# danielSanchezQ/dkg

Measured on AMD Instinct MI355X. Metric: verified shares/sec (whole node) at n=1024,t=511; full-ceremony wall time, higher is better.
Workload: dtype u32 (GF(2^255-19), Z_l); 1 GPU; one DKG ceremony n=1024, t=511 (share gen + round-2/4 checks + finalise); n=1024, t=511, parallelism=single GPU, verify_streams=2, rounds_2_4_fused=True, degree_split=4, recombination=short lattice multipliers, recombination_addends=affine Niels, stepping_additions=dedicated (complete redo where exceptional)

## Files before the change

### dkg_amd/csrc/ge25519.h

```cpp
#pragma once
#include "fe25519.h"

struct ge_p3 {
  fe X, Y, Z, T;
};
struct ge_cached {
  fe YpX, YmX, Z2, T2d;
};
struct ge_aff {
  fe ypx, ymx, xy2d;
};

namespace ge_const {
__device__ static const uint32_t D[10] = {0x35978a3u, 0xd37284u, 0x3156ebdu, 0x6a0a0eu, 0x1c029u,
                                          0x179e898u, 0x3a03cbbu, 0x1ce7198u, 0x2e2b6ffu, 0x1480db3u};
__device__ static const uint32_t D2[10] = {0x2b2f159u, 0x1a6e509u, 0x22add7au, 0xd4141du, 0x38052u,
                                           0xf3d130u, 0x3407977u, 0x19ce331u, 0x1c56dffu, 0x901b67u};
__device__ static const uint32_t D4[10] = {0x165e2b2u, 0x14dca13u, 0x55baf5u, 0x1a8283bu, 0x700a4u,
                                           0x1e7a260u, 0x280f2eeu, 0x139c663u, 0x38adbffu, 0x12036ceu};
__device__ static const uint32_t D16[10] = {0x1978aeeu, 0x137284du, 0x156ebd6u, 0xa0a0ecu, 0x1c0293u,
                                            0x19e8980u, 0x203cbbbu, 0xe7198eu, 0x22b6ffeu, 0x80db3bu};
__device__ static const uint32_t SQRT_M1[10] = {0x20ea0b0u, 0x186c9d2u, 0x8f189du, 0x35697fu,
                                                0xbd0c60u, 0x1fbd7a7u, 0x2804c9eu, 0x1e16569u,
                                                0x4fc1du, 0xae0c92u};
__device__ static const uint32_t SQRT_AD_MINUS_ONE[10] = {
    0x17b2e1bu, 0x1fda812u, 0x297afd2u, 0x60dbc2u, 0x2be7638u,
    0x1f5d1fdu, 0x27e6498u, 0x11581e7u, 0x3f2b834u, 0xdda4c6u};
__device__ static const uint32_t INVSQRT_A_MINUS_D[10] = {
    0x5d40eau, 0x3f6aa0u, 0x257d339u, 0xbad20bu, 0x274bc58u,
    0x1d840u, 0x13dc8ffu, 0x19442d8u, 0x5cfaffu, 0x1e1b224u};
__device__ static const uint32_t ONE_MINUS_D_SQ[10] = {
    0x5fc176u, 0x1027065u, 0x2a1fc4fu, 0x1c66af1u, 0xb20684u,
    0x70dfe4u, 0x255eedfu, 0x1af332u, 0x28b2b3eu, 0xa41cau};
__device__ static const uint32_t D_MINUS_ONE_SQ[10] = {
    0xed4d20u, 0x156aa91u, 0x3332635u, 0x16580f0u, 0x34a7928u,
    0x9b4eebu, 0x26997a9u, 0x48299bu, 0x3af66c2u, 0x165a2cdu};
}

DKG_DEV void fe_ld(fe& r, const uint32_t* c) {
#pragma unroll
  for (int i = 0; i < 10; i++) r.v[i] = c[i];
}

DKG_DEV void ge_identity(ge_p3& p) {
  fe_zero(p.X);
  fe_one(p.Y);
  fe_one(p.Z);
  fe_zero(p.T);
}

DKG_DEV void ge_to_cached(ge_cached& c, const ge_p3& p) {
  fe_add(c.YpX, p.Y, p.X);
  fe_sub(c.YmX, p.Y, p.X);
  fe_dbl(c.Z2, p.Z);
  fe d2;
  fe_ld(d2, ge_const::D2);
  fe_mul(c.T2d, p.T, d2);
}

DKG_DEV void ge_cached_neg(ge_cached& r, const ge_cached& c) {
  fe_copy(r.YpX, c.YmX);
  fe_copy(r.YmX, c.YpX);
  fe_copy(r.Z2, c.Z2);
  fe_neg(r.T2d, c.T2d);
  fe_carry(r.T2d, r.T2d);
}

template <bool IL = false>
DKG_DEV void ge_add(ge_p3& r, const ge_p3& p, const ge_cached& q) {
  if constexpr (IL && DKG_PW) {
    fe a, b, e, h, t, u;
    fe_sub(t, p.Y, p.X);
    fe_add(u, p.Y, p.X);
    fe_mul2(a, t, q.YmX, b, u, q.YpX);
    fe_sub(e, b, a);
    fe_add(h, b, a);
    fe_mul2(a, p.T, q.T2d, b, p.Z, q.Z2);
    fe_sub(t, b, a);
    fe_add(b, b, a);
    fe_mul2(r.X, e, t, r.Y, b, h);
    fe_mul2(r.Z, b, t, r.T, e, h);
    return;
  }
  fe a, b, e, h, t;
  fe_sub(t, p.Y, p.X);
  fe_mul(a, t, q.YmX);
  fe_add(t, p.Y, p.X);
  fe_mul(b, t, q.YpX);
  fe_sub(e, b, a);
  fe_add(h, b, a);
  fe_mul(a, p.T, q.T2d);
  fe_mul(b, p.Z, q.Z2);
  fe_sub(t, b, a);
  fe_add(b, b, a);
  fe_mul(r.X, e, t);
  fe_mul(r.Y, b, h);
  fe_mul(r.Z, b, t);
  fe_mul(r.T, e, h);
}

DKG_DEV void ge_sub(ge_p3& r, const ge_p3& p, const ge_cached& q) {
  fe a, b, e, h, t;
  fe_sub(t, p.Y, p.X);
  fe_mul(a, t, q.YpX);
// ... 144 lines not shown
    fe_add(h, a, b);
    fe_sub(g, a, b);
    fe_add(a, p.X, p.Y);
    fe_sq2(t, p.Z, a, a);
    fe_dbl(t, t);
    fe_add(t, t, g);
    fe_carry(t, t);
    fe_sub(b, h, a);
    fe_mul2(r.X, b, t, r.Y, g, h);
    if (with_t) fe_mul2(r.Z, g, t, r.T, b, h);
    else fe_mul(r.Z, g, t);
    return;
  }
  fe a, b, t, h, g;
  fe_sq(a, p.X);
  fe_sq(b, p.Y);
  fe_add(h, a, b);
  fe_sub(g, a, b);
  fe_sq(t, p.Z);
  fe_dbl(t, t);
  fe_add(t, t, g);
  fe_carry(t, t);
  fe_add(a, p.X, p.Y);
  fe_sq(a, a);
  fe_sub(b, h, a);
  fe_mul(r.X, b, t);
  fe_mul(r.Y, g, h);
  fe_mul(r.Z, g, t);
  if (with_t) fe_mul(r.T, b, h);
}

template <bool IL = false>
DKG_DEV void ge_add_signed(ge_p3& r, const ge_p3& p, const ge_cached& q, bool neg, bool with_t = true) {
  fe a, b, e, h, t, qa, qb;
#pragma unroll
  for (int i = 0; i < 10; i++) {
    qa.v[i] = neg ? q.YpX.v[i] : q.YmX.v[i];
    qb.v[i] = neg ? q.YmX.v[i] : q.YpX.v[i];
  }
  if constexpr (IL && DKG_PW) {
    fe u;
    fe_sub(t, p.Y, p.X);
    fe_add(u, p.Y, p.X);
    fe_mul2(a, t, qa, b, u, qb);
  } else {
    fe_sub(t, p.Y, p.X);
    fe_mul(a, t, qa);
    fe_add(t, p.Y, p.X);
    fe_mul(b, t, qb);
  }
  fe_sub(e, b, a);
  fe_add(h, b, a);
  if constexpr (IL && DKG_PW) {
    fe_mul2(a, p.T, q.T2d, b, p.Z, q.Z2);
  } else {
    fe_mul(a, p.T, q.T2d);
    fe_mul(b, p.Z, q.Z2);
  }
  fe na;
  fe_neg(na, a);
  fe_cmov(a, na, neg);
  fe_sub(t, b, a);
  fe_add(b, b, a);
  if constexpr (IL && DKG_PW) {
    fe_mul2(r.X, e, t, r.Y, b, h);
    if (with_t) fe_mul2(r.Z, b, t, r.T, e, h);
    else fe_mul(r.Z, b, t);
  } else {
    fe_mul(r.X, e, t);
    fe_mul(r.Y, b, h);
    fe_mul(r.Z, b, t);
    if (with_t) fe_mul(r.T, e, h);
  }
}

template <bool IL = false>
DKG_DEV void ge_madd_signed(ge_p3& r, const ge_p3& p, const ge_aff& q, bool neg, bool with_t = true) {
  fe a, b, e, h, t, qa, qb;
#pragma unroll
  for (int i = 0; i < 10; i++) {
    qa.v[i] = neg ? q.ypx.v[i] : q.ymx.v[i];
    qb.v[i] = neg ? q.ymx.v[i] : q.ypx.v[i];
  }
  if constexpr (IL && DKG_PW) {
    fe u;
    fe_sub(t, p.Y, p.X);
    fe_add(u, p.Y, p.X);
    fe_mul2(a, t, qa, b, u, qb);
  } else {
    fe_sub(t, p.Y, p.X);
    fe_mul(a, t, qa);
    fe_add(t, p.Y, p.X);
    fe_mul(b, t, qb);
  }
  fe_sub(e, b, a);
  fe_add(h, b, a);
  fe_mul(a, p.T, q.xy2d);
  fe na;
  fe_neg(na, a);
  fe_cmov(a, na, neg);
  fe_dbl(b, p.Z);
  fe_carry(b, b);
  fe_sub(t, b, a);
  fe_add(b, b, a);
  if constexpr (IL && DKG_PW) {
    fe_mul2(r.X, e, t, r.Y, b, h);
    if (with_t) fe_mul2(r.Z, b, t, r.T, e, h);
    else fe_mul(r.Z, b, t);
  } else {
    fe_mul(r.X, e, t);
    fe_mul(r.Y, b, h);
    fe_mul(r.Z, b, t);
    if (with_t) fe_mul(r.T, e, h);
  }
}

template <bool IL = false>
DKG_DEV void ge_madd_swapped(ge_p3& r, const ge_p3& p, const ge_aff& q, bool neg, bool with_t = true) {
  fe a, b, e, h, t;
  const fe& qa = q.ymx;
  const fe& qb = q.ypx;
  if constexpr (IL && DKG_PW) {
    fe u;
    fe_sub(t, p.Y, p.X);
    fe_add(u, p.Y, p.X);
    fe_mul2(a, t, qa, b, u, qb);
  } else {
    fe_sub(t, p.Y, p.X);
    fe_mul(a, t, qa);
    fe_add(t, p.Y, p.X);
    fe_mul(b, t, qb);
  }
  fe_sub(e, b, a);
  fe_add(h, b, a);
  fe_mul(a, p.T, q.xy2d);
  fe na;
  fe_neg(na, a);
  fe_cmov(a, na, neg);
  fe_dbl(b, p.Z);
  fe_carry(b, b);
  fe_sub(t, b, a);
  fe_add(b, b, a);
  if constexpr (IL && DKG_PW) {
    fe_mul2(r.X, e, t, r.Y, b, h);
    if (with_t) fe_mul2(r.Z, b, t, r.T, e, h);
    else fe_mul(r.Z, b, t);
  } else {
    fe_mul(r.X, e, t);
    fe_mul(r.Y, b, h);
    fe_mul(r.Z, b, t);
    if (with_t) fe_mul(r.T, e, h);
  }
}


DKG_DEV bool fe_sqrt_ratio_m1(fe& r, const fe& u, const fe& v) {
  fe v3, v7, t, chk, neg_u, neg_u_i, sqrtm1;
  fe_ld(sqrtm1, ge_const::SQRT_M1);
  fe_sq(v3, v);
  fe_mul(v3, v3, v);
  fe_sq(v7, v3);
  fe_mul(v7, v7, v);
  fe_mul(t, u, v7);
  fe_pow22523(t, t);
  fe_mul(t, t, v3);
  fe_mul(r, t, u);
  fe_sq(chk, r);
  fe_mul(chk, chk, v);
  fe_neg(neg_u, u);
  fe_carry(neg_u, neg_u);
  fe_mul(neg_u_i, neg_u, sqrtm1);
  fe d;
  fe_sub(d, chk, u);
  bool correct = fe_iszero(d);
  fe_sub(d, chk, neg_u);
  bool flipped = fe_iszero(d);
  fe_sub(d, chk, neg_u_i);
  bool flipped_i = fe_iszero(d);
  fe r_prime;
  fe_mul(r_prime, r, sqrtm1);
  fe_cmov(r, r_prime, flipped || flipped_i);
  fe_abs(r, r);
  return correct || flipped;
}

DKG_DEV void fe_sq_x2(fe (&r)[2], const fe (&a)[2]) { fe_sq2(r[0], a[0], r[1], a[1]); }
DKG_DEV void fe_mul_x2(fe (&r)[2], const fe (&a)[2], const fe (&b)[2]) {
  fe_mul2(r[0], a[0], b[0], r[1], a[1], b[1]);
}
DKG_DEV void fe_sqn_x2(fe (&r)[2], const fe (&a)[2], int n) {
  fe_sq_x2(r, a);
  for (int i = 1; i < n; i++) fe_sq_x2(r, r);
}
DKG_DEV void fe_pow22523_x2(fe (&out)[2], const fe (&z)[2]) {
  fe t0[2], t1[2], t2[2];
  fe_sq_x2(t0, z);
  fe_sqn_x2(t1, t0, 2);
  fe_mul_x2(t1, z, t1);
  fe_mul_x2(t0, t0, t1);
  fe_sq_x2(t0, t0);
  fe_mul_x2(t0, t1, t0);
  fe_sqn_x2(t1, t0, 5);
  fe_mul_x2(t0, t1, t0);
  fe_sqn_x2(t1, t0, 10);
// ... 201 lines not shown
```

### dkg_amd/csrc/kernels.hip

```cpp
#ifdef DKG_FE_ILP
#define dkgk dkgk_ilp
#endif
#include "kernels.h"
#include "split.h"

#include <algorithm>
#include <cmath>
#include <type_traits>
#include "points.h"

namespace dkgk {

constexpr int COMB_WORDS = AFF_WORDS * COMB_ENTRIES;

#ifndef DKG_DECODE_WAVES
#define DKG_DECODE_WAVES 2
#endif
__global__ __launch_bounds__(256, DKG_DECODE_WAVES) void k_decode(const uint32_t* __restrict__ comp, size_t count,
                                                uint32_t* __restrict__ ext, size_t stride,
                                                uint8_t* __restrict__ ok, size_t pm_N, size_t pm_npad,
                                                uint32_t nseg, uint32_t seg, size_t pm_L, size_t pm_pstride) {
  size_t e = (size_t)blockIdx.x * blockDim.x + threadIdx.x;
  if (e >= count) return;
  uint32_t w[8];
// ... 1712 lines not shown
  const uint32_t* dw = digits + j * 256;
  const uint32_t* dw1 = digits + (nrecv + j) * 256;
  const int tp = top[j];
  ge_p3 acc;
  ge_identity(acc);
#pragma unroll 1
  for (int b = tp; b >= 0; b--) {
    uint64_t w = (uint32_t)__builtin_amdgcn_readfirstlane(dw[b]);
    if constexpr (K > 4) w |= (uint64_t)(uint32_t)__builtin_amdgcn_readfirstlane(dw1[b]) << 32;
    if (b != tp) ge_dbl_lean<DKG_AFF_IL != 0>(acc, acc, w != 0 || b == 0);
    aff_position<0, K, KL>(acc, w, qs, qr, b == 0);
  }
  if (live) pt_store_aos<DKG_COMB_NT != 0>(R, c * nrecv + j, acc);
}

void combine_short_aff(size_t width, size_t pstride, size_t pieces, size_t nrecv, const uint32_t* digits,
                       const int16_t* top, const uint32_t* A, uint32_t* R, hipStream_t stream, size_t j0, size_t jn) {
  if (!jn) jn = nrecv - j0;
  if (!width || !jn || pieces < 2 || pieces > 5) return;
  const dim3 grid((unsigned)((width + 63) / 64), (unsigned)jn);
  if (pieces == 2)
    hipLaunchKernelGGL((k_combine_aff<2, 1>), grid, dim3(64), 0, stream, width, pstride, nrecv, digits, top, A, R, j0);
  else if (pieces == 3)
    hipLaunchKernelGGL((k_combine_aff<3, 2>), grid, dim3(64), 0, stream, width, pstride, nrecv, digits, top, A, R, j0);
  else if (pieces == 4)
    hipLaunchKernelGGL((k_combine_aff<4, 2>), grid, dim3(64), 0, stream, width, pstride, nrecv, digits, top, A, R, j0);
  else
    hipLaunchKernelGGL((k_combine_aff<5, 2>), grid, dim3(64), 0, stream, width, pstride, nrecv, digits, top, A, R, j0);
}

constexpr int AFFQ_RUN = 32;

DKG_DEV void ld_zt(fe& z, fe& t, const uint32_t* R, size_t e) {
  const uint4* p4 = reinterpret_cast<const uint4*>(R + e * PT_WORDS) + 5;
  const uint4 a = p4[0], b = p4[1], c = p4[2], d = p4[3], f = p4[4];
  z = fe{{a.x, a.y, a.z, a.w, b.x, b.y, b.z, b.w, c.x, c.y}};
  t = fe{{c.z, c.w, d.x, d.y, d.z, d.w, f.x, f.y, f.z, f.w}};
}
DKG_DEV void ld_xy(fe& x, fe& y, const uint32_t* R, size_t e) {
  const uint4* p4 = reinterpret_cast<const uint4*>(R + e * PT_WORDS);
  const uint4 a = p4[0], b = p4[1], c = p4[2], d = p4[3], f = p4[4];
  x = fe{{a.x, a.y, a.z, a.w, b.x, b.y, b.z, b.w, c.x, c.y}};
  y = fe{{c.z, c.w, d.x, d.y, d.z, d.w, f.x, f.y, f.z, f.w}};
}
template <bool SC>
DKG_DEV void pair_fg(fe& z01, fe& f, fe& g, const fe& z0, const fe& t0, const fe& z1, const fe& t1, const fe& dc) {
  fe c, d;
  fe_mul(z01, z0, z1);
  fe_mul(c, t0, t1);
  fe_mul(c, c, dc);
  if constexpr (SC) {
    fe_copy(d, z01);
  } else {
    fe_dbl(d, z01);
    fe_carry(d, d);
  }
  fe_sub(f, d, c);
  fe_add(g, d, c);
}
DKG_DEV void st_niels(uint32_t* slot, const fe& x, const fe& y, const fe& d2) {
  fe ypx, ymx, t;
  fe_mul(t, x, y);
  fe_mul(t, t, d2);
  fe_add(ypx, y, x);
  fe_sub(ymx, y, x);
  st_fe3(slot, ypx, ymx, t);
}

template <bool SC>
__global__ __launch_bounds__(256) __attribute__((amdgpu_waves_per_eu(2, 2))) void k_affine_pairs(size_t width, size_t pstride, size_t pieces, size_t nrecv,
                                                      const uint32_t* __restrict__ R, uint32_t* __restrict__ A,
                                                      size_t j0, size_t jn, unsigned ls, unsigned rl) {
  const size_t span = (size_t)ls * rl, runs = (jn + span - 1) / span;
  const size_t gid = (size_t)blockIdx.x * blockDim.x + threadIdx.x;
  const size_t item = gid / ls;
  if (item >= (pieces / 2) * width * runs) return;
  const size_t c = item % width, rest = item / width, run = rest % runs, p = rest / runs;
  const size_t plane = pstride * nrecv;
  const size_t e0 = (2 * p * pstride + c) * nrecv + j0;
  const size_t jb = run * span + (gid % ls);
  const int cnt = jb < jn ? (int)min((size_t)rl, (jn - jb + ls - 1) / ls) : 0;
  auto pt = [&](int i) { return e0 + jb + ls * (size_t)i; };
  fe d2, dc;
  fe_ld(d2, ge_const::D2);
  fe_ld(dc, SC ? ge_const::D16 : ge_const::D2);
  fe acc;
  fe_one(acc);
#pragma unroll 1
  for (int i = 0; i < cnt; i++) {
    uint4* a4 = reinterpret_cast<uint4*>(A + pt(i) * AFFP_WORDS);
    a4[0] = make_uint4(acc.v[0], acc.v[1], acc.v[2], acc.v[3]);
    a4[1] = make_uint4(acc.v[4], acc.v[5], acc.v[6], acc.v[7]);
    a4[2] = make_uint4(acc.v[8], acc.v[9], 0u, 0u);
    fe z0, t0, z1, t1, z01, f, g;
    ld_zt(z0, t0, R, pt(i));
    ld_zt(z1, t1, R, pt(i) + plane);
    pair_fg<SC>(z01, f, g, z0, t0, z1, t1, dc);
    fe_mul(acc, acc, z01);
    fe_mul(f, f, g);
    fe_mul(acc, acc, f);
  }
  fe inv;
  fe_invert(inv, acc);
  if constexpr (SC) {
    fe_dbl(inv, inv);
    fe_carry(inv, inv);
  }
#pragma unroll 1
  for (int i = cnt - 1; i >= 0; i--) {
    const size_t e = pt(i);
    uint32_t* slot = A + e * AFFP_WORDS;
    fe z0, t0, z1, t1, z01, f, g, zs, iz0, iz1;
    ld_zt(z0, t0, R, e);
    ld_zt(z1, t1, R, e + plane);
    pair_fg<SC>(z01, f, g, z0, t0, z1, t1, dc);
    fe_mul(zs, f, g);
    {
      const uint4* a4 = reinterpret_cast<const uint4*>(slot);
      const uint4 q0 = a4[0], q1 = a4[1], q2 = a4[2];
      const fe pre = {{q0.x, q0.y, q0.z, q0.w, q1.x, q1.y, q1.z, q1.w, q2.x, q2.y}};
      fe t, i01;
      fe_mul(t, inv, pre);
      fe_mul(inv, inv, z01);
      fe_mul(inv, inv, zs);
      fe_mul(i01, t, zs);
      fe_mul(zs, t, z01);
      fe_mul(iz0, i01, z1);
      fe_mul(iz1, i01, z0);
    }
    fe_mul(f, f, zs);
    fe_mul(g, g, zs);
    fe ym0, yp0, ym1, yp1;
    {
      fe X, Y, x, y;
      ld_xy(X, Y, R, e);
      fe_sub(ym0, Y, X);
      fe_add(yp0, Y, X);
      fe_mul(x, X, iz0);
      fe_mul(y, Y, iz0);
      st_niels(slot, x, y, d2);
      ld_xy(X, Y, R, e + plane);
      fe_sub(ym1, Y, X);
      fe_add(yp1, Y, X);
      fe_mul(x, X, iz1);
      fe_mul(y, Y, iz1);
      st_niels(slot + plane * AFFP_WORDS, x, y, d2);
    }
    fe a, b, eh, x, y;
    fe_mul(a, ym0, ym1);
    fe_mul(b, yp0, yp1);
    fe_sub(eh, b, a);
    fe_mul(x, eh, f);
    fe_add(eh, b, a);
    fe_mul(y, eh, g);
    st_niels(slot + pieces * plane * AFFP_WORDS, x, y, d2);
    fe_mul(a, ym0, yp1);
    fe_mul(b, yp0, ym1);
    fe_sub(eh, b, a);
    fe_mul(x, eh, g);
    fe_add(eh, b, a);
    fe_mul(y, eh, f);
    st_niels(slot + (pieces + 1) * plane * AFFP_WORDS, x, y, d2);
  }
}

void affine_pairs(size_t width, size_t pstride, size_t pieces, size_t nrecv, const uint32_t* R, uint32_t* A,
                  hipStream_t stream, size_t j0, size_t jn, bool scaled) {
  if (!jn) jn = nrecv - j0;
  if (!width || !jn || pieces < 2) return;
  unsigned rl = AFFQ_RUN;
  while (rl > 8 && (pieces / 2) * width * ((jn + rl - 1) / rl) < 65536) rl /= 2;
  unsigned ls = 32;
  while (ls > 1 && (size_t)(ls / 2) * rl >= jn) ls /= 2;
  const size_t runs = (jn + (size_t)ls * rl - 1) / ((size_t)ls * rl), lanes = (pieces / 2) * width * runs * ls;
  hipLaunchKernelGGL(scaled ? k_affine_pairs<true> : k_affine_pairs<false>, dim3((unsigned)((lanes + 255) / 256)),
                     dim3(256), 0, stream, width, pstride, pieces, nrecv, R, A, j0, jn, ls, rl);
}

DKG_DEV void jsf_fetch(ge_aff& q, const uint32_t* __restrict__ A0, uint32_t slot, size_t plane, uint32_t e) {
  if (e == JSF_EV_NONE) return;
  asm volatile("" : "+v"(slot));
  const uint32_t* a = A0 + (size_t)slot * AFFP_WORDS + (e & 3u) * plane;
  const uint2* f0 = reinterpret_cast<const uint2*>(a + ((e & 4u) ? 10 : 0));
  const uint2* f1 = reinterpret_cast<const uint2*>(a + ((e & 4u) ? 0 : 10));
  const uint2* f2 = reinterpret_cast<const uint2*>(a + 20);
#pragma unroll
  for (int i = 0; i < 5; i++) {
    const uint2 u = f0[i], v = f1[i], w = f2[i];
    q.ypx.v[2 * i] = u.x;
    q.ypx.v[2 * i + 1] = u.y;
    q.ymx.v[2 * i] = v.x;
    q.ymx.v[2 * i + 1] = v.y;
    q.xy2d.v[2 * i] = w.x;
    q.xy2d.v[2 * i + 1] = w.y;
  }
}

struct JsfStream {
  ge_aff q;
  const uint32_t* A0;
  uint32_t slot;
  size_t plane;
  const uint32_t* ev;
  uint32_t next;
  int k;
};

template <int P, int K, int KL>
DKG_DEV void jsf_position(ge_p3& acc, uint32_t w, const uint32_t* qs, const ge_aff* qr, JsfStream& s, bool last) {
  if constexpr (2 * P < K) {
    const int e0 = (int8_t)(w >> (16 * P)), e1 = (int8_t)(w >> (16 * P + 8));
    bool t = last;
    if constexpr (2 * P + 2 < K) t = t || (w >> (16 * P + 16)) != 0;
    if (e0 != 0 && e1 != 0) {
      ge_madd_swapped<DKG_AFF_IL != 0>(acc, acc, s.q, e0 < 0, t);
      const uint32_t e = s.next;
      s.next = (uint32_t)__builtin_amdgcn_readfirstlane(s.ev[s.k]);
      s.k++;
      jsf_fetch(s.q, s.A0, s.slot, s.plane, e);
    } else if (e0 != 0 || e1 != 0) {
      constexpr int U0 = 2 * P, U1 = 2 * P + 1;
      if constexpr (U1 < KL) {
        const int u = e0 != 0 ? U0 : U1;
        ge_madd_lds<DKG_AFF_IL != 0>(acc, acc, qs + u * AFF_WORDS * 64 + threadIdx.x, (e0 | e1) < 0, 64, t);
      } else if (e0 != 0) {
        if constexpr (U0 < KL) ge_madd_lds<DKG_AFF_IL != 0>(acc, acc, qs + U0 * AFF_WORDS * 64 + threadIdx.x, e0 < 0, 64, t);
        else ge_madd_signed<DKG_AFF_IL != 0>(acc, acc, qr[U0 - KL], e0 < 0, t);
      } else {
        ge_madd_signed<DKG_AFF_IL != 0>(acc, acc, qr[U1 - KL], e1 < 0, t);
      }
    }
    jsf_position<P + 1, K, KL>(acc, w, qs, qr, s, last);
  }
}

template <int K, int KL>
__global__ __launch_bounds__(64, 2) void k_combine_jsf(size_t width, size_t pstride, size_t nrecv,
                                                       const uint32_t* __restrict__ digits,
                                                       const int16_t* __restrict__ top,
                                                       const uint32_t* __restrict__ ev,
                                                       const uint32_t* __restrict__ A, uint32_t* __restrict__ R,
                                                       size_t j0) {
  static_assert(K % 2 == 0 && K <= 4, "whole pairs in one digit word");
  __shared__ uint32_t qs[KL * AFF_WORDS * 64];
  const size_t c = (size_t)blockIdx.x * 64 + threadIdx.x;
  const size_t j = j0 + blockIdx.y;
  const bool live = c < width;
  const size_t cc = live ? c : 0;
  ge_aff qr[K - KL > 0 ? K - KL : 1];
  aff_addends<0, K, KL>(qs, qr, A, pstride, cc, nrecv, j);
  const uint32_t* dw = digits + j * 256;
  const int tp = top[j];
  JsfStream s;
  s.A0 = A + ((size_t)K * pstride * nrecv + j) * AFFP_WORDS;
  s.slot = (uint32_t)(cc * nrecv);
  s.plane = pstride * nrecv * AFFP_WORDS;
  s.ev = ev + j * JSF_EV_WORDS;
  s.next = (uint32_t)__builtin_amdgcn_readfirstlane(s.ev[1]);
  s.k = 2;
#pragma unroll
  for (int u = 0; u < K - KL; u++) {
#pragma unroll
    for (int i = 0; i < 10; i++)
      asm volatile("" : "+v"(qr[u].ypx.v[i]), "+v"(qr[u].ymx.v[i]), "+v"(qr[u].xy2d.v[i]));
  }
  fe_zero(s.q.ypx);
  fe_zero(s.q.ymx);
  fe_zero(s.q.xy2d);
  jsf_fetch(s.q, s.A0, s.slot, s.plane, (uint32_t)__builtin_amdgcn_readfirstlane(s.ev[0]));
  ge_p3 acc;
  ge_identity(acc);
#pragma unroll 1
  for (int b = tp; b >= 0; b--) {
    const uint32_t w = (uint32_t)__builtin_amdgcn_readfirstlane(dw[b]);
    if (b != tp) ge_dbl_lean<DKG_AFF_IL != 0>(acc, acc, w != 0 || b == 0);
    jsf_position<0, K, KL>(acc, w, qs, qr, s, b == 0);
  }
  if (live) pt_store_aos<DKG_COMB_NT != 0>(R, (size_t)s.slot + j, acc);
}

void combine_short_jsf(size_t width, size_t pstride, size_t pieces, size_t nrecv, const uint32_t* digits,
                       const int16_t* top, const uint32_t* ev, const uint32_t* A, uint32_t* R, hipStream_t stream,
                       size_t j0, size_t jn) {
  if (!jn) jn = nrecv - j0;
  if (!width || !jn || (pieces != 2 && pieces != 4)) return;
  const dim3 grid((unsigned)((width + 63) / 64), (unsigned)jn);
  if (pieces == 2)
    hipLaunchKernelGGL((k_combine_jsf<2, 1>), grid, dim3(64), 0, stream, width, pstride, nrecv, digits, top, ev, A, R, j0);
  else
    hipLaunchKernelGGL((k_combine_jsf<4, 2>), grid, dim3(64), 0, stream, width, pstride, nrecv, digits, top, ev, A, R, j0);
}

void combine(size_t width, size_t pstride, size_t pieces, size_t nrecv, const int8_t* digits, const int16_t* top,
             uint32_t* R, hipStream_t stream) {
  if (!width || !nrecv || pieces < 2) return;
  const dim3 grid((unsigned)((width + 63) / 64), (unsigned)nrecv);
  if (pieces == 2)
    hipLaunchKernelGGL(k_combine<1>, grid, dim3(64), 0, stream, width, pstride, (int)pieces, nrecv, digits, top, R);
  else
    hipLaunchKernelGGL(k_combine<2>, grid, dim3(64), 0, stream, width, pstride, (int)pieces, nrecv, digits, top, R);
}

__global__ __launch_bounds__(256, DKG_COMB_WAVES) void k_check(size_t ndealers, size_t nrecv, size_t dealer_base, size_t recv_base,
                                               uint32_t nmod, int round,
                                               const uint32_t* __restrict__ s, const uint32_t* __restrict__ sp,
                                               const uint32_t* __restrict__ R,
                                               const uint32_t* __restrict__ tab_g,
                                               const uint32_t* __restrict__ tab_h,
                                               const uint8_t* __restrict__ dok, uint8_t* __restrict__ dec,
                                               const uint32_t* __restrict__ scale) {
  const size_t p = (size_t)blockIdx.x * blockDim.x + threadIdx.x;
  if (p >= ndealers * nrecv) return;
  const size_t i = p / nrecv, j = p % nrecv;
  ge_p3 acc, r;
  ge_identity(acc);
  sc x, f;
  if (scale) sc_load(f, scale + 8 * j);
  sc_load(x, s + 8 * p);
  if (scale) sc_mont_mul(x, x, f);
  combw_mul_add(acc, x, tab_g);
  if (round == 2) {
    sc_load(x, sp + 8 * p);
    if (scale) sc_mont_mul(x, x, f);
    combw_mul_add(acc, x, tab_h);
  }
  pt_load_aos(r, R, p);
  const bool eq = ristretto_eq(acc, r);
  uint8_t v = dok[i] ? (eq ? 1 : 0) : (round == 2 ? 4 : 0);
  if ((uint32_t)((i + dealer_base) % nmod) == (uint32_t)(j + recv_base)) v = 2;
  dec[p] = v;
}

void check(size_t ndealers, size_t nrecv, size_t dealer_base, size_t recv_base, size_t nmod, int round,
           const uint32_t* s, const uint32_t* sp, const uint32_t* R, const uint32_t* tab_g,
           const uint32_t* tab_h, const uint8_t* dok, uint8_t* dec, hipStream_t stream, const uint32_t* scale) {
  const size_t total = ndealers * nrecv;
  if (!total) return;
  hipLaunchKernelGGL(k_check, dim3((unsigned)((total + 255) / 256)), dim3(256), 0, stream, ndealers, nrecv,
                     dealer_base, recv_base, (uint32_t)nmod, round, s, sp, R, tab_g, tab_h, dok, dec, scale);
}

template <int PASS>
__global__ __launch_bounds__(256, DKG_COMB_WAVES) void k_check_both(size_t ndealers, size_t nrecv, size_t dealer0, size_t dealer_base,
                                                    uint32_t nmod, const uint32_t* __restrict__ s,
                                                    const uint32_t* __restrict__ sp, const uint32_t* __restrict__ R,
                                                    const uint32_t* __restrict__ tab_g,
                                                    const uint32_t* __restrict__ tab_h,
                                                    const uint8_t* __restrict__ dok, uint8_t* __restrict__ dec2,
                                                    uint8_t* __restrict__ dec4, const uint32_t* __restrict__ scale,
                                                    size_t j0, size_t jn, uint32_t* __restrict__ accb) {
  const size_t p = (size_t)blockIdx.x * blockDim.x + threadIdx.x;
  if (p >= ndealers * jn) return;
  const size_t i = dealer0 + p / jn, j = j0 + p % jn;
  const size_t cE = (i / 64) * 128 + i % 64, cA = cE + 64;
  const size_t q = i * nrecv + j;
  const bool self = (uint32_t)((i + dealer_base) % nmod) == (uint32_t)j;
  ge_p3 acc, r;
  sc x, f;
  if (scale) sc_load(f, scale + 8 * j);
  if constexpr (PASS != 2) {
    ge_identity(acc);
// ... 591 lines not shown
```

### dkg_amd/csrc/points.h

```cpp
#pragma once
#include "ge25519.h"
#include "sc25519.h"

constexpr int PT_WORDS = 40;
constexpr int AFF_WORDS = 30;
constexpr int COMB_ENTRIES = 512;

DKG_DEV void pt_load(ge_p3& p, const uint32_t* __restrict__ base, size_t stride, size_t e) {
#pragma unroll
  for (int i = 0; i < 10; i++) {
    p.X.v[i] = base[(size_t)(i)*stride + e];
    p.Y.v[i] = base[(size_t)(10 + i) * stride + e];
    p.Z.v[i] = base[(size_t)(20 + i) * stride + e];
    p.T.v[i] = base[(size_t)(30 + i) * stride + e];
  }
}

DKG_DEV void pt_store(uint32_t* __restrict__ base, size_t stride, size_t e, const ge_p3& p) {
#pragma unroll
  for (int i = 0; i < 10; i++) {
    base[(size_t)(i)*stride + e] = p.X.v[i];
    base[(size_t)(10 + i) * stride + e] = p.Y.v[i];
    base[(size_t)(20 + i) * stride + e] = p.Z.v[i];
    base[(size_t)(30 + i) * stride + e] = p.T.v[i];
// ... 260 lines not shown
  fe_sub(e, b, a);
  fe_add(h, b, a);
  lds_get_fe(qv, q, 3, stride);
  fe_mul(a, p.T, qv);
  if (neg) fe_neg(a, a);
  lds_get_fe(qv, q, 2, stride);
  fe_mul(b, p.Z, qv);
  fe_sub(t, b, a);
  fe_add(b, b, a);
  fe_mul(r.X, e, t);
  fe_mul(r.Y, b, h);
  fe_mul(r.Z, b, t);
  if (with_t) fe_mul(r.T, e, h);
}

DKG_DEV void ge_to_cached_ded(ge_cached& c, const ge_p3& p) {
  fe_add(c.YpX, p.Y, p.X);
  fe_sub(c.YmX, p.Y, p.X);
  fe_dbl(c.Z2, p.Z);
  fe_dbl(c.T2d, p.T);
}
DKG_DEV void ge_add_ded_lds(ge_p3& r, const ge_p3& p, const uint32_t* q, int stride = 64) {
#if DKG_FE_PAIR && !defined(DKG_FE_ILP)
  fe a, b, e, h, t, u, qv, qw;
  fe_sub(t, p.Y, p.X);
  lds_get_fe(qv, q, 0, stride);
  fe_add(u, p.Y, p.X);
  lds_get_fe(qw, q, 1, stride);
  fe_mul2(a, t, qv, b, u, qw);
  fe_sub(e, b, a);
  fe_add(h, b, a);
  lds_get_fe(qv, q, 3, stride);
  lds_get_fe(qw, q, 2, stride);
  fe_mul2(a, p.Z, qv, b, p.T, qw);
  fe_add(t, b, a);
  fe_sub(b, b, a);
  fe_mul2(r.X, t, e, r.T, t, b);
  fe_mul2(r.Y, h, b, r.Z, h, e);
#else
  fe a, b, e, h, t, qv;
  fe_sub(t, p.Y, p.X);
  lds_get_fe(qv, q, 0, stride);
  fe_mul(a, t, qv);
  fe_add(t, p.Y, p.X);
  lds_get_fe(qv, q, 1, stride);
  fe_mul(b, t, qv);
  fe_sub(e, b, a);
  fe_add(h, b, a);
  lds_get_fe(qv, q, 3, stride);
  fe_mul(a, p.Z, qv);
  lds_get_fe(qv, q, 2, stride);
  fe_mul(b, p.T, qv);
  fe_add(t, b, a);
  fe_sub(b, b, a);
  fe_mul(r.X, t, e);
  fe_mul(r.Y, h, b);
  fe_mul(r.T, t, b);
  fe_mul(r.Z, h, e);
#endif
}

DKG_DEV void ge_to_scaled(ge_p3& s, const ge_p3& p) {
  fe_dbl(s.X, p.X);
  fe_carry(s.X, s.X);
  fe_dbl(s.Y, p.Y);
  fe_carry(s.Y, s.Y);
  fe_dbl(s.Z, p.Z);
  fe_carry(s.Z, s.Z);
  fe_dbl(s.Z, s.Z);
  fe_carry(s.Z, s.Z);
  fe_copy(s.T, p.T);
}
DKG_DEV void ge_to_cached_sc(ge_cached& c, const ge_p3& s) {
  fe_add(c.YpX, s.Y, s.X);
  fe_sub(c.YmX, s.Y, s.X);
  fe_copy(c.Z2, s.Z);
  fe_copy(c.T2d, s.T);
}
DKG_DEV void ge_add_sc_lds(ge_p3& r, const ge_p3& p, const uint32_t* q, int stride = 64) {
  ge_add_ded_lds(r, p, q, stride);
}

template <bool IL = false>
DKG_DEV void ge_add_ded_lds_s(ge_p3& r, const ge_p3& p, const uint32_t* q, bool neg, int stride = 64,
                              bool with_t = true) {
  if constexpr (IL && DKG_PW) {
    fe a, b, e, h, t, u, qv, qw;
    fe_sub(t, p.Y, p.X);
    lds_get_fe(qv, q, neg ? 1 : 0, stride);
    fe_add(u, p.Y, p.X);
    lds_get_fe(qw, q, neg ? 0 : 1, stride);
    fe_mul2(a, t, qv, b, u, qw);
    fe_sub(e, b, a);
    fe_add(h, b, a);
    lds_get_fe(qv, q, 3, stride);
    lds_get_fe(qw, q, 2, stride);
    fe_mul2(a, p.Z, qv, b, p.T, qw);
    if (neg) fe_neg(a, a);
    fe_add(t, b, a);
    fe_sub(b, b, a);
    fe_mul2(r.X, t, e, r.Y, h, b);
    if (with_t) fe_mul2(r.Z, h, e, r.T, t, b);
    else fe_mul(r.Z, h, e);
    return;
  }
  fe a, b, e, h, t, qv;
  fe_sub(t, p.Y, p.X);
  lds_get_fe(qv, q, neg ? 1 : 0, stride);
  fe_mul(a, t, qv);
  fe_add(t, p.Y, p.X);
  lds_get_fe(qv, q, neg ? 0 : 1, stride);
  fe_mul(b, t, qv);
  fe_sub(e, b, a);
  fe_add(h, b, a);
  lds_get_fe(qv, q, 3, stride);
  fe_mul(a, p.Z, qv);
  if (neg) fe_neg(a, a);
  lds_get_fe(qv, q, 2, stride);
  fe_mul(b, p.T, qv);
  fe_add(t, b, a);
  fe_sub(b, b, a);
  fe_mul(r.X, t, e);
  fe_mul(r.Y, h, b);
  fe_mul(r.Z, h, e);
  if (with_t) fe_mul(r.T, t, b);
}

template <bool IL = false>
DKG_DEV void ge_madd_lds(ge_p3& r, const ge_p3& p, const uint32_t* q, bool neg, int stride = 64,
                         bool with_t = true) {
  if constexpr (IL && DKG_PW) {
    fe a, b, e, h, t, u, qv, qw;
    fe_sub(t, p.Y, p.X);
    lds_get_fe(qv, q, neg ? 0 : 1, stride);
    fe_add(u, p.Y, p.X);
    lds_get_fe(qw, q, neg ? 1 : 0, stride);
    fe_mul2(a, t, qv, b, u, qw);
    fe_sub(e, b, a);
    fe_add(h, b, a);
    lds_get_fe(qv, q, 2, stride);
    fe_mul(a, p.T, qv);
    if (neg) fe_neg(a, a);
    fe_dbl(b, p.Z);
    fe_carry(b, b);
    fe_sub(t, b, a);
    fe_add(b, b, a);
    fe_mul2(r.X, e, t, r.Y, b, h);
    if (with_t) fe_mul2(r.Z, b, t, r.T, e, h);
    else fe_mul(r.Z, b, t);
    return;
  }
  fe a, b, e, h, t, qv;
  fe_sub(t, p.Y, p.X);
  lds_get_fe(qv, q, neg ? 0 : 1, stride);
  fe_mul(a, t, qv);
  fe_add(t, p.Y, p.X);
  lds_get_fe(qv, q, neg ? 1 : 0, stride);
  fe_mul(b, t, qv);
  fe_sub(e, b, a);
  fe_add(h, b, a);
  lds_get_fe(qv, q, 2, stride);
  fe_mul(a, p.T, qv);
  if (neg) fe_neg(a, a);
  fe_dbl(b, p.Z);
  fe_carry(b, b);
  fe_sub(t, b, a);
// ... 8 lines not shown
```

Before: 12.92 million verified shares/s.

## Use scaled point representation in JSF combine loop with unified addend selection

Switches the short-lattice JSF recombination accumulator to a scaled extended-coordinate form (Z doubled, T scaled) so mixed additions skip the 2Z doubling and conditional negation, and doublings use a leaner formula. Affine addend precomputation now folds the scale into xy2d (using 16d and a multiply by 1/2 instead of doubling the inverse). The recursive per-position template dispatch is replaced by a runtime loop that gathers the addend into one ge_aff and calls a single madd, which cuts code size but adds register copies and dynamic selection over register-held addends. The result is converted back to standard form before storing.

After: 13.00 million verified shares/s (median of 6 runs). No clear change (+0.6%).

```diff
diff --git a/dkg_amd/csrc/ge25519.h b/dkg_amd/csrc/ge25519.h
--- a/dkg_amd/csrc/ge25519.h
+++ b/dkg_amd/csrc/ge25519.h
@@ -20,6 +20,8 @@
                                            0x1e7a260u, 0x280f2eeu, 0x139c663u, 0x38adbffu, 0x12036ceu};
 __device__ static const uint32_t D16[10] = {0x1978aeeu, 0x137284du, 0x156ebd6u, 0xa0a0ecu, 0x1c0293u,
                                             0x19e8980u, 0x203cbbbu, 0xe7198eu, 0x22b6ffeu, 0x80db3bu};
+__device__ static const uint32_t HALF[10] = {0x3fffff7u, 0x1ffffffu, 0x3ffffffu, 0x1ffffffu, 0x3ffffffu,
+                                             0x1ffffffu, 0x3ffffffu, 0x1ffffffu, 0x3ffffffu, 0xffffffu};
 __device__ static const uint32_t SQRT_M1[10] = {0x20ea0b0u, 0x186c9d2u, 0x8f189du, 0x35697fu,
                                                 0xbd0c60u, 0x1fbd7a7u, 0x2804c9eu, 0x1e16569u,
                                                 0x4fc1du, 0xae0c92u};
@@ -330,44 +332,6 @@
     qa.v[i] = neg ? q.ypx.v[i] : q.ymx.v[i];
     qb.v[i] = neg ? q.ymx.v[i] : q.ypx.v[i];
   }
-  if constexpr (IL && DKG_PW) {
-    fe u;
-    fe_sub(t, p.Y, p.X);
-    fe_add(u, p.Y, p.X);
-    fe_mul2(a, t, qa, b, u, qb);
-  } else {
-    fe_sub(t, p.Y, p.X);
-    fe_mul(a, t, qa);
-    fe_add(t, p.Y, p.X);
-    fe_mul(b, t, qb);
-  }
-  fe_sub(e, b, a);
-  fe_add(h, b, a);
-  fe_mul(a, p.T, q.xy2d);
-  fe na;
-  fe_neg(na, a);
-  fe_cmov(a, na, neg);
-  fe_dbl(b, p.Z);
-  fe_carry(b, b);
-  fe_sub(t, b, a);
-  fe_add(b, b, a);
-  if constexpr (IL && DKG_PW) {
-    fe_mul2(r.X, e, t, r.Y, b, h);
-    if (with_t) fe_mul2(r.Z, b, t, r.T, e, h);
-    else fe_mul(r.Z, b, t);
-  } else {
-    fe_mul(r.X, e, t);
-    fe_mul(r.Y, b, h);
-    fe_mul(r.Z, b, t);
-    if (with_t) fe_mul(r.T, e, h);
-  }
-}
-
-template <bool IL = false>
-DKG_DEV void ge_madd_swapped(ge_p3& r, const ge_p3& p, const ge_aff& q, bool neg, bool with_t = true) {
-  fe a, b, e, h, t;
-  const fe& qa = q.ymx;
-  const fe& qb = q.ypx;
   if constexpr (IL && DKG_PW) {
     fe u;
     fe_sub(t, p.Y, p.X);
diff --git a/dkg_amd/csrc/kernels.hip b/dkg_amd/csrc/kernels.hip
--- a/dkg_amd/csrc/kernels.hip
+++ b/dkg_amd/csrc/kernels.hip
@@ -1818,7 +1818,7 @@
   const int cnt = jb < jn ? (int)min((size_t)rl, (jn - jb + ls - 1) / ls) : 0;
   auto pt = [&](int i) { return e0 + jb + ls * (size_t)i; };
   fe d2, dc;
-  fe_ld(d2, ge_const::D2);
+  fe_ld(d2, ge_const::D16);
   fe_ld(dc, SC ? ge_const::D16 : ge_const::D2);
   fe acc;
   fe_one(acc);
@@ -1838,9 +1838,10 @@
   }
   fe inv;
   fe_invert(inv, acc);
-  if constexpr (SC) {
-    fe_dbl(inv, inv);
-    fe_carry(inv, inv);
+  if constexpr (!SC) {
+    fe half;
+    fe_ld(half, ge_const::HALF);
+    fe_mul(inv, inv, half);
   }
 #pragma unroll 1
   for (int i = cnt - 1; i >= 0; i--) {
@@ -1942,32 +1943,41 @@
   int k;
 };
 
-template <int P, int K, int KL>
-DKG_DEV void jsf_position(ge_p3& acc, uint32_t w, const uint32_t* qs, const ge_aff* qr, JsfStream& s, bool last) {
-  if constexpr (2 * P < K) {
-    const int e0 = (int8_t)(w >> (16 * P)), e1 = (int8_t)(w >> (16 * P + 8));
-    bool t = last;
-    if constexpr (2 * P + 2 < K) t = t || (w >> (16 * P + 16)) != 0;
-    if (e0 != 0 && e1 != 0) {
-      ge_madd_swapped<DKG_AFF_IL != 0>(acc, acc, s.q, e0 < 0, t);
-      const uint32_t e = s.next;
-      s.next = (uint32_t)__builtin_amdgcn_readfirstlane(s.ev[s.k]);
-      s.k++;
-      jsf_fetch(s.q, s.A0, s.slot, s.plane, e);
-    } else if (e0 != 0 || e1 != 0) {
-      constexpr int U0 = 2 * P, U1 = 2 * P + 1;
-      if constexpr (U1 < KL) {
-        const int u = e0 != 0 ? U0 : U1;
-        ge_madd_lds<DKG_AFF_IL != 0>(acc, acc, qs + u * AFF_WORDS * 64 + threadIdx.x, (e0 | e1) < 0, 64, t);
-      } else if (e0 != 0) {
-        if constexpr (U0 < KL) ge_madd_lds<DKG_AFF_IL != 0>(acc, acc, qs + U0 * AFF_WORDS * 64 + threadIdx.x, e0 < 0, 64, t);
-        else ge_madd_signed<DKG_AFF_IL != 0>(acc, acc, qr[U0 - KL], e0 < 0, t);
-      } else {
-        ge_madd_signed<DKG_AFF_IL != 0>(acc, acc, qr[U1 - KL], e1 < 0, t);
+template <int K, int KL>
+DKG_DEV void jsf_addend(ge_aff& q, int pr, int e0, int e1, const uint32_t* qs, const ge_aff* qr, JsfStream& s) {
+  bool neg;
+  if (e0 != 0 && e1 != 0) {
+    neg = e0 < 0;
+    fe_copy(q.ypx, s.q.ypx);
+    fe_copy(q.ymx, s.q.ymx);
+    fe_copy(q.xy2d, s.q.xy2d);
+    const uint32_t e = s.next;
+    s.next = (uint32_t)__builtin_amdgcn_readfirstlane(s.ev[s.k]);
+    s.k++;
+    jsf_fetch(s.q, s.A0, s.slot, s.plane, e);
+  } else {
+    const int u = 2 * pr + (e0 == 0);
+    neg = (e0 | e1) < 0;
+    if (u < KL) {
+      const uint32_t* l = qs + u * AFF_WORDS * 64 + threadIdx.x;
+      lds_get_fe(q.ypx, l, neg ? 1 : 0);
+      lds_get_fe(q.ymx, l, neg ? 0 : 1);
+      lds_get_fe(q.xy2d, l, 2);
+    } else {
+#pragma unroll
+      for (int v = 0; v < K - KL; v++) {
+        if (u == KL + v) {
+#pragma unroll
+          for (int i = 0; i < 10; i++) {
+            q.ypx.v[i] = neg ? qr[v].ymx.v[i] : qr[v].ypx.v[i];
+            q.ymx.v[i] = neg ? qr[v].ypx.v[i] : qr[v].ymx.v[i];
+            q.xy2d.v[i] = qr[v].xy2d.v[i];
+          }
+        }
       }
     }
-    jsf_position<P + 1, K, KL>(acc, w, qs, qr, s, last);
-  }
+  }
+  if (neg) fe_neg(q.xy2d, q.xy2d);
 }
 
 template <int K, int KL>
@@ -2005,14 +2015,24 @@
   fe_zero(s.q.xy2d);
   jsf_fetch(s.q, s.A0, s.slot, s.plane, (uint32_t)__builtin_amdgcn_readfirstlane(s.ev[0]));
   ge_p3 acc;
-  ge_identity(acc);
+  ge_identity_sc(acc);
 #pragma unroll 1
   for (int b = tp; b >= 0; b--) {
-    const uint32_t w = (uint32_t)__builtin_amdgcn_readfirstlane(dw[b]);
-    if (b != tp) ge_dbl_lean<DKG_AFF_IL != 0>(acc, acc, w != 0 || b == 0);
-    jsf_position<0, K, KL>(acc, w, qs, qr, s, b == 0);
-  }
-  if (live) pt_store_aos<DKG_COMB_NT != 0>(R, (size_t)s.slot + j, acc);
+    uint32_t w = (uint32_t)__builtin_amdgcn_readfirstlane(dw[b]);
+    if (b != tp) ge_dbl_sc<DKG_AFF_IL != 0>(acc, acc, w != 0 || b == 0);
+#pragma unroll 1
+    for (int pr = 0; pr < K / 2; pr++, w >>= 16) {
+      const int e0 = (int8_t)w, e1 = (int8_t)(w >> 8);
+      if (e0 == 0 && e1 == 0) continue;
+      ge_aff q;
+      jsf_addend<K, KL>(q, pr, e0, e1, qs, qr, s);
+      ge_madd_sc<DKG_AFF_IL != 0>(acc, acc, q, b == 0 || (2 * pr + 2 < K && (w >> 16) != 0));
+    }
+  }
+  if (live) {
+    ge_from_scaled(acc, acc);
+    pt_store_aos<DKG_COMB_NT != 0>(R, (size_t)s.slot + j, acc);
+  }
 }
 
 void combine_short_jsf(size_t width, size_t pstride, size_t pieces, size_t nrecv, const uint32_t* digits,
diff --git a/dkg_amd/csrc/points.h b/dkg_amd/csrc/points.h
--- a/dkg_amd/csrc/points.h
+++ b/dkg_amd/csrc/points.h
@@ -366,6 +366,86 @@
 }
 
 template <bool IL = false>
+DKG_DEV void ge_madd_sc(ge_p3& r, const ge_p3& p, const ge_aff& q, bool with_t = true) {
+  fe a, b, e, h, t;
+  if constexpr (IL && DKG_PW) {
+    fe u;
+    fe_sub(t, p.Y, p.X);
+    fe_add(u, p.Y, p.X);
+    fe_mul2(a, t, q.ymx, b, u, q.ypx);
+  } else {
+    fe_sub(t, p.Y, p.X);
+    fe_mul(a, t, q.ymx);
+    fe_add(t, p.Y, p.X);
+    fe_mul(b, t, q.ypx);
+  }
+  fe_sub(e, b, a);
+  fe_add(h, b, a);
+  fe_mul(a, p.T, q.xy2d);
+  fe_sub(t, p.Z, a);
+  fe_add(b, p.Z, a);
+  if constexpr (IL && DKG_PW) {
+    fe_mul2(r.X, e, t, r.Y, b, h);
+    if (with_t) fe_mul2(r.Z, b, t, r.T, e, h);
+    else fe_mul(r.Z, b, t);
+  } else {
+    fe_mul(r.X, e, t);
+    fe_mul(r.Y, b, h);
+    fe_mul(r.Z, b, t);
+    if (with_t) fe_mul(r.T, e, h);
+  }
+}
+template <bool IL = false>
+DKG_DEV void ge_dbl_sc(ge_p3& r, const ge_p3& p, bool with_t) {
+  fe a, b, t, h, g;
+  if constexpr (IL && DKG_PW) {
+    fe_sq2(a, p.X, b, p.Y);
+    fe_add(h, a, b);
+    fe_sub(g, a, b);
+    fe_dbl(g, g);
+    fe_add(a, p.X, p.Y);
+    fe_sq2(t, p.Z, a, a);
+    fe_add(t, t, g);
+    fe_carry(t, t);
+    fe_sub(b, h, a);
+    fe_mul2(r.X, b, t, r.Y, g, h);
+    if (with_t) fe_mul2(r.Z, g, t, r.T, b, h);
+    else fe_mul(r.Z, g, t);
+    return;
+  }
+  fe_sq(a, p.X);
+  fe_sq(b, p.Y);
+  fe_add(h, a, b);
+  fe_sub(g, a, b);
+  fe_dbl(g, g);
+  fe_sq(t, p.Z);
+  fe_add(t, t, g);
+  fe_carry(t, t);
+  fe_add(a, p.X, p.Y);
+  fe_sq(a, a);
+  fe_sub(b, h, a);
+  fe_mul(r.X, b, t);
+  fe_mul(r.Y, g, h);
+  fe_mul(r.Z, g, t);
+  if (with_t) fe_mul(r.T, b, h);
+}
+DKG_DEV void ge_identity_sc(ge_p3& s) {
+  ge_identity(s);
+  s.Z.v[0] = 2;
+}
+DKG_DEV void ge_from_scaled(ge_p3& p, const ge_p3& s) {
+  fe_dbl(p.X, s.X);
+  fe_carry(p.X, p.X);
+  fe_dbl(p.Y, s.Y);
+  fe_carry(p.Y, p.Y);
+  fe_copy(p.Z, s.Z);
+  fe_dbl(p.T, s.T);
+  fe_carry(p.T, p.T);
+  fe_dbl(p.T, p.T);
+  fe_carry(p.T, p.T);
+}
+
+template <bool IL = false>
 DKG_DEV void ge_add_ded_lds_s(ge_p3& r, const ge_p3& p, const uint32_t* q, bool neg, int stride = 64,
                               bool with_t = true) {
   if constexpr (IL && DKG_PW) {
```
